# tigrazone/zig_raytracing_contest

Measured on AMD Instinct MI355X. Metric: Mrays/sec + wall-clock to output.png on contest config.json scene, higher is better.
Workload: dtype f32; 1 GPU; cfg3: contest stand-in (99480 tris, 553091 refs), 1920x1080, 256 spp, max_bounce 4, grid 128^3; global_batch=530841600, parallelism=tiles1, schedule=timed: default pass sets

## Files before the change

### zig_raytracing_contest_amd/csrc/render.hip

```cpp
#include <hip/hip_runtime.h>

#include <algorithm>
#include <cstdio>
#include <cstdlib>
#include <cstring>
#include <ctime>
#include <new>
#include <vector>

#include "zrt_internal.h"
#include "dda.h"
#include "escape.h"
#include "device_geometry.h"

using namespace zrt;

#define HIP_TRY(expr)                                                            \
    do {                                                                         \
        hipError_t _e = (expr);                                                  \
        if (_e != hipSuccess) {                                                  \
            if (getenv("ZRT_DEBUG"))                                             \
                fprintf(stderr, "zrt: %s failed: %s (%s:%d)\n", #expr,           \
                        hipGetErrorString(_e), __FILE__, __LINE__);              \
            return _e == hipErrorOutOfMemory ? ZRT_ERR_OUT_OF_MEMORY : ZRT_ERR_HIP; \
        }                                                                        \
    } while (0)

namespace {

constexpr float kFltEps = 1.1920928955078125e-07f;
constexpr int kBlock = 256;
constexpr int kTraceBlock = 512;
constexpr int kTraceThreads = 256;
#ifndef ZRT_TRI_BATCH
#define ZRT_TRI_BATCH 1
#endif
constexpr int kTriBatch = ZRT_TRI_BATCH;
#ifndef ZRT_PARK_BLOCK_T
#define ZRT_PARK_BLOCK_T 1024
#endif
constexpr int kParkBlock = ZRT_PARK_BLOCK_T;
#ifndef ZRT_SHADE_N
#define ZRT_SHADE_N 3
#endif
constexpr int kShadeEntries = ZRT_SHADE_N;
#ifndef ZRT_WF_CHUNK
#define ZRT_WF_CHUNK 3
#endif
constexpr uint32_t kWfChunk = ZRT_WF_CHUNK;

#ifndef ZRT_PLANES16
#define ZRT_PLANES16 1
#endif
#ifndef ZRT_ESCAPE
#define ZRT_ESCAPE 1
#endif
#ifndef ZRT_FRUSTUM
#define ZRT_FRUSTUM 1
#endif
#ifndef ZRT_FRUSTUM_HI
#define ZRT_FRUSTUM_HI 1
#endif
#ifndef ZRT_NORMALIZE_RN
#define ZRT_NORMALIZE_RN 1
#endif
#if ZRT_NORMALIZE_RN
#define ZRT_NORM_RN normalize_rn
#else
#define ZRT_NORM_RN normalize
#endif
#ifndef ZRT_FFN
#define ZRT_FFN 1
#endif
#ifndef ZRT_PRIMARY_BMASK
#define ZRT_PRIMARY_BMASK 1
#endif
#ifndef ZRT_WALK_FACE_SKIP
#define ZRT_WALK_FACE_SKIP 1
#endif
#ifndef ZRT_FAST_QUOT_WF
#define ZRT_FAST_QUOT_WF 1
#endif
#ifndef ZRT_FRUSTUM_SHIFT
#define ZRT_FRUSTUM_SHIFT 2
#endif
constexpr uint32_t kFrustShift = ZRT_FRUSTUM_SHIFT;
static_assert(kFrustShift <= 3, "a frustum block lies inside one tile (tile edges are multiples of 8)");
#ifndef ZRT_PACK_BM
#define ZRT_PACK_BM 1
#endif

constexpr double kFrustB = (double)(1u << ZRT_FRUSTUM_SHIFT);
#ifndef ZRT_WALK_STEPS
#define ZRT_WALK_STEPS 4
#endif
#ifndef ZRT_WALK_STEPS_NOESC
#define ZRT_WALK_STEPS_NOESC 5
#endif
constexpr uint32_t kTriFloats = 12u;

struct TraceParams {
    float bmin[3], bmax[3];
    uint32_t res[3];
    float cs[3];
    float ics[3];
    uint32_t cs_ok;
    const uint2* cells;
    const float* tri_pos;
    const float4* tri_data;
    const DevMat* mats;
    uint32_t nmat;
    const float* texels;
    const double* zig;
    const uint32_t* occ;
    uint32_t occ_shift, occ_nb0, occ_nb01, occ_words;
    const unsigned long long* bmask;
    const float4* tlo;
    uint32_t tlo_nbx;
    PackK pk;
    const uint32_t* cell32;
    uint32_t occ_o1, occ_o2, occ_w0, occ_w1, occ_w2, occ_lowm;
    uint32_t ox1, ox2, ow0, ow1, ow2;
    float org[3], llc[3], right[3], up[3];
    uint32_t w;
    const uint32_t* pixlist;
    uint32_t P;
    uint32_t s0;
    uint32_t total;
    uint32_t S;
    DivS sdiv;
    uint32_t max_bounce;
    uint64_t seed;
    float4* out;
    uint32_t* counter;
    unsigned long long* stats;
};

__device__ __forceinline__ void load_tri(const TraceParams& p, uint32_t j, v3& v0, v3& e1, v3& e2) {
    const float* q = p.tri_pos + (uint64_t)kTriFloats * j;
    const float4 a = *reinterpret_cast<const float4*>(q), b = *reinterpret_cast<const float4*>(q + 4),
                 c = *reinterpret_cast<const float4*>(q + 8);
    v0 = mk(a.x, a.y, a.z); e1 = mk(b.x, b.y, b.z); e2 = mk(c.x, c.y, c.z);
}

template <int N>
struct Stack {
    float e[3 * N], a[3 * N];
    uint32_t used;
    __device__ __forceinline__ void init() { used = 0u; }
    __device__ __forceinline__ void set(uint32_t slot, v3 ee, v3 aa) {
        e[3 * slot] = ee.x; e[3 * slot + 1] = ee.y; e[3 * slot + 2] = ee.z;
        a[3 * slot] = aa.x; a[3 * slot + 1] = aa.y; a[3 * slot + 2] = aa.z;
        used |= 1u << slot;
    }
    __device__ __forceinline__ v3 fold(v3 L) const {
        for (int i = N - 1; i >= 0; --i) {
            if ((used >> i) & 1u) {
                L = add(mk(e[3 * i], e[3 * i + 1], e[3 * i + 2]),
                        mul(mk(a[3 * i], a[3 * i + 1], a[3 * i + 2]), L));
            }
        }
        return L;
    }
};

__device__ __forceinline__ bool brick_occupied(const TraceParams& p, const uint32_t* occ, uint32_t c0,
                                               uint32_t c1, uint32_t c2) {
    const uint32_t s = p.occ_shift;
    const uint32_t b = __umul24(c2 >> s, p.occ_nb01) + __umul24(c1 >> s, p.occ_nb0) + (c0 >> s);
    return (occ[b >> 5] >> (b & 31u)) & 1u;
}

template <bool BM>
__device__ __forceinline__ bool brick_occupied_v(const TraceParams& p, const uint32_t* occ, uint32_t pc) {
    if (BM) {
        return __builtin_amdgcn_ubfe(occ[pc >> 11], pc >> 6, 1u);
    }
    const uint32_t b = __umul24(__builtin_amdgcn_ubfe(pc, p.occ_o2, p.occ_w2), p.occ_nb01) +
                       __umul24(__builtin_amdgcn_ubfe(pc, p.occ_o1, p.occ_w1), p.occ_nb0) +
                       __builtin_amdgcn_ubfe(pc, p.occ_shift, p.occ_w0);
    return (occ[b >> 5] >> (b & 31u)) & 1u;
}

template <bool BM>
__device__ __forceinline__ bool occx_cell(unsigned long long bm, const DdaV& s, const PackK& k) {
    if (BM) return (uint32_t)(bm >> (s.pc & 63u)) & 1u;
    const uint32_t i = __umul24(s.pc & k.low2, k.kmul) >> k.kshr;
    return (uint32_t)(bm >> (i & 63u)) & 1u;
}

__device__ __forceinline__ GridK grid_consts(const TraceParams& p) {
    GridK g;
    g.rm0 = __builtin_amdgcn_readfirstlane(p.res[0] - 1u);
    g.rm1 = __builtin_amdgcn_readfirstlane(p.res[1] - 1u);
    g.rm2 = __builtin_amdgcn_readfirstlane(p.res[2] - 1u);
    g.str1 = __builtin_amdgcn_readfirstlane(p.res[0]);
    g.str2 = __builtin_amdgcn_readfirstlane(p.res[0] * p.res[1]);
    return g;
}

__device__ __forceinline__ bool first_active_lane() {
    return (threadIdx.x & 63u) == (uint32_t)__builtin_ctzll(__ballot(1));
}

template <int TB, bool STATS, bool MTX = false>
__device__ __forceinline__ void test_cell(const TraceParams& p, uint32_t b, uint32_t e, v3 o, v3 d,
                                          float& nearest, float& hu, float& hv, uint32_t& hidx,
                                          uint32_t& n_tests, uint64_t* wstat) {
    for (uint32_t i = b; i < e; i += TB) {
        if (STATS && first_active_lane()) ++wstat[1];
        v3 A[TB], B[TB], Cc[TB];
#pragma unroll
        for (int k = 0; k < TB; ++k) load_tri(p, min(i + (uint32_t)k, e - 1u), A[k], B[k], Cc[k]);
#pragma unroll
        for (int k = 0; k < TB; ++k) {
            if (i + (uint32_t)k < e) {
                if (STATS) ++n_tests;
                float t, u, v;
                if (tri_ray<MTX>(A[k], B[k], Cc[k], o, d, &t, &u, &v)) {
                    if (nearest > t && t > 0.0f) { nearest = t; hu = u; hv = v; hidx = i + k; }
                }
            }
        }
    }
}

template <int TB, bool MTX>
__device__ __forceinline__ void test_cell_keep(const TraceParams& p, uint32_t b, uint32_t e, uint32_t keep, v3 o,
                                               v3 d, float& nearest, float& hu, float& hv, uint32_t& hidx) {
    const uint32_t cnt = e - b;
    if (cnt > 32u || keep == ~0u) {
        uint32_t dummy = 0;
        test_cell<TB, false, MTX>(p, b, e, o, d, nearest, hu, hv, hidx, dummy, nullptr);
        return;
    }
    uint32_t m = keep & ((cnt < 32u ? (1u << cnt) : 0u) - 1u);
    while (m) {
        uint32_t k[TB];
        bool has[TB];
#pragma unroll
        for (int j = 0; j < TB; ++j) {
            has[j] = m != 0u;
            k[j] = has[j] ? (uint32_t)__builtin_ctz(m) : k[0];
            m &= m - 1u;
        }
        v3 A[TB], B[TB], Cc[TB];
#pragma unroll
        for (int j = 0; j < TB; ++j) load_tri(p, b + k[j], A[j], B[j], Cc[j]);
#pragma unroll
        for (int j = 0; j < TB; ++j) {
            if (has[j]) {
                float t, u, v;
                if (tri_ray<MTX>(A[j], B[j], Cc[j], o, d, &t, &u, &v)) {
                    if (nearest > t && t > 0.0f) { nearest = t; hu = u; hv = v; hidx = b + k[j]; }
                }
            }
        }
    }
}

template <bool STATS, int TB, bool PACKED = false, bool PK_BM = false, bool MTX = false>
__device__ __forceinline__ float trace_ray(const TraceParams& p, const uint32_t* occ, v3 o, v3 d,
                                           float& hu, float& hv, uint32_t& hidx, uint32_t& n_cells,
                                           uint32_t& n_tests, uint64_t* prof, uint32_t* wcnt = nullptr,
                                           float tau = 0.0f, float tfar = kInf) {
    float nearest = kInf;
    Dda s0;
    if (ZRT_FAST_QUOT && ZRT_FAST_QUOT_WF && !MTX && !STATS) {
        if (!dda_init_fq(p.bmin, p.bmax, p.res, p.cs, p.ics, p.cs_ok != 0u, o, d, s0)) return nearest;
    } else if (!dda_init(p.bmin, p.bmax, p.res, p.cs, o, d, s0)) {
        return nearest;
    }
    const uint32_t sh = p.occ_shift;
    const GridK gk = grid_consts(p);
    if constexpr (PACKED) {
        static_assert(!STATS, "the counting build walks unpacked");
        DdaV s;
        ddav_from_t<PK_BM>(s0, gk, p.pk, s);
        uint32_t f0 = p.pk.f0, f1 = p.pk.f1, f2 = p.pk.f2;
        asm("" : "+s"(f0), "+s"(f1), "+s"(f2));
        if (ZRT_FRUSTUM && s0.neg < 8u) {
            if (tau == kInf) return nearest;
            if (tau > fminf(s.tn0, fminf(s.tn1, s.tn2))) {
                bool exited;
                if (ZRT_FFN) DDAV_FFN(s, p.pk, f0, f1, f2, tau, exited);
                else DDAV_FF4(s, f0, f1, f2, tau, exited);
                if (exited) return nearest;
            }
        }
        bool occupied = brick_occupied_v<PK_BM>(p, occ, s.pc);
        constexpr bool kBm = PK_BM && ZRT_PRIMARY_BMASK;
        unsigned long long q = 0ull;
        if (kBm && occupied) q = p.bmask[s.pc >> 6];
        float lim = ZRT_FRUSTUM_HI && s0.neg < 8u ? tfar : kInf;
        float tcl = __builtin_nanf("");
        for (;;) {
            if (kBm ? ((q >> (s.pc & 63u)) & 1ull) != 0ull : occupied) {
                const uint32_t* rec = p.cell32 + 8ull * s.pc;
                const uint2 cell = *reinterpret_cast<const uint2*>(rec);
                if (ZRT_WALK_FACE_SKIP) {
                    const bool x0 = s.tn0 == tcl + s.td0, x1 = s.tn1 == tcl + s.td1, x2 = s.tn2 == tcl + s.td2;
                    uint32_t keep = ~0u;
                    if ((uint32_t)x0 + (uint32_t)x1 + (uint32_t)x2 == 1u) {
                        const uint32_t face = x0 ? (s.d0 >> 31) : (x1 ? 2u + (s.d1 >> 31) : 4u + (s.d2 >> 31));
                        keep = rec[2 + face];
                    }
                    test_cell_keep<TB, MTX>(p, cell.x, cell.y, keep, o, d, nearest, hu, hv, hidx);
                } else {
                    test_cell<TB, false, MTX>(p, cell.x, cell.y, o, d, nearest, hu, hv, hidx, n_tests, prof);
                }
                lim = fminf(lim, nearest);
            }
            bool crossed, exited;
            float tc;
            PackK pkl = p.pk;
            pkl.f0 = f0; pkl.f1 = f1; pkl.f2 = f2;
            DDAV_STEPX(s, pkl, p.occ_lowm, crossed, exited, tc);
            if (exited || lim <= tc) break;
            tcl = tc;
            if (crossed) {
                occupied = brick_occupied_v<PK_BM>(p, occ, s.pc);
                if (kBm) q = occupied ? p.bmask[s.pc >> 6] : 0ull;
            }
        }
        return nearest;
    }
    DdaW s;
    ddaw_from(s0, gk, s);
    bool occupied = brick_occupied(p, occ, s.c0, s.c1, s.c2);
    for (;;) {
        if (STATS) ++n_cells;
        if (STATS && first_active_lane()) ++prof[8];
        uint32_t ncell = 0;
        if (occupied) {
            const uint2 cell = p.cells[s.lin];
            if (STATS) { prof[6] += 1; prof[7] += cell.y > cell.x ? 1 : 0; ncell = cell.y - cell.x; }
            test_cell<TB, STATS, MTX>(p, cell.x, cell.y, o, d, nearest, hu, hv, hidx, n_tests, prof + 8);
        }
        if (STATS) {
            uint32_t* wc = wcnt + 2 * (threadIdx.x >> 6);
            const bool first = first_active_lane();
            if (first) wc[0] = 0;
            __builtin_amdgcn_wave_barrier();
            atomicAdd(&wc[0], ncell);
            __builtin_amdgcn_wave_barrier();
            if (first) {
                const uint32_t N = wc[0];
                prof[10] += N ? 1 : 0;
                prof[4] += (N + 63) / 64;
            }
        }
        bool crossed;
        float t_exit;
        DDAW_STEP(s, sh, crossed, t_exit);
        if (nearest <= t_exit) break;
        if (crossed) occupied = brick_occupied(p, occ, s.c0, s.c1, s.c2);
    }
    return nearest;
}

#ifndef ZRT_TEX1
#define ZRT_TEX1 1
#endif
__device__ __forceinline__ v3 sample3(const float* texels, const DevTex& t, float u, float v) {
    const float* b = texels + t.off;
    if (ZRT_TEX1 && t.w == 1 && t.h == 1) {
        const float fu = tex_frac(u), fv = tex_frac(v);
        const float x = __int_as_float(t.umin), y = __int_as_float(t.umax), z = __int_as_float(t.vmin);
        return mk(bilerp(x, x, x, x, fu, fv), bilerp(y, y, y, y, fu, fv), bilerp(z, z, z, z, fu, fv));
    }
    const TexCoords c = tex_coords(t.w, t.h, t.umin, t.umax, t.vmin, t.vmax, u, v);
    v3 r;
    r.x = bilerp(b[3 * c.i11 + 0], b[3 * c.i21 + 0], b[3 * c.i12 + 0], b[3 * c.i22 + 0], c.fu, c.fv);
    r.y = bilerp(b[3 * c.i11 + 1], b[3 * c.i21 + 1], b[3 * c.i12 + 1], b[3 * c.i22 + 1], c.fu, c.fv);
    r.z = bilerp(b[3 * c.i11 + 2], b[3 * c.i21 + 2], b[3 * c.i12 + 2], b[3 * c.i22 + 2], c.fu, c.fv);
    return r;
}
__device__ __forceinline__ float sample1(const float* texels, const DevTex& t, float u, float v) {
    const float* b = texels + t.off;
    if (ZRT_TEX1 && t.w == 1 && t.h == 1) {
        const float x = __int_as_float(t.umin);
        return bilerp(x, x, x, x, tex_frac(u), tex_frac(v));
    }
    const TexCoords c = tex_coords(t.w, t.h, t.umin, t.umax, t.vmin, t.vmax, u, v);
    return bilerp(b[c.i11], b[c.i21], b[c.i12], b[c.i22], c.fu, c.fv);
}

__device__ __forceinline__ unsigned long long wave_sum(unsigned long long x) {
#pragma unroll
    for (int off = 32; off > 0; off >>= 1) {
        const unsigned lo = __shfl_xor((unsigned)x, off);
        const unsigned hi = __shfl_xor((unsigned)(x >> 32), off);
        x += ((unsigned long long)hi << 32) | lo;
    }
    return x;
}

__device__ __forceinline__ void camera_ray(const TraceParams& p, uint32_t item, Rng& rng, v3& o, v3& d,
                                           uint32_t* block = nullptr) {
    const uint32_t q = div_by(item, p.sdiv);
    const uint32_t s_local = item - q * p.S;
    const uint32_t pixel = p.pixlist[q];
    const uint32_t py = pixel / p.w;
    const uint32_t px = pixel - py * p.w;
    if (block) *block = (py >> kFrustShift) * p.tlo_nbx + (px >> kFrustShift);
    rng.s = path_key(p.seed, pixel, p.s0 + s_local);
    const float jx = rng_float(rng);
    const float jy = rng_float(rng);
    o = mk(p.org[0], p.org[1], p.org[2]);
    d = ZRT_NORM_RN(add(add(mk(p.llc[0], p.llc[1], p.llc[2]),
                          scale(mk(p.right[0], p.right[1], p.right[2]), (float)px + jx)),
                      scale(mk(p.up[0], p.up[1], p.up[2]), (float)py + jy)));
}

__device__ __forceinline__ Rng camera_rng(const TraceParams& p, uint32_t item) {
    const uint32_t q = div_by(item, p.sdiv);
    const uint32_t s_local = item - q * p.S;
    const uint32_t pixel = p.pixlist[q];
    Rng rng;
    rng.s = path_key(p.seed, pixel, p.s0 + s_local);
    (void)rng_float(rng);
    (void)rng_float(rng);
    return rng;
}

template <int MAXB>
__global__ __launch_bounds__(kTraceBlock, 1) void trace_kernel(const TraceParams p) {
    __shared__ double s_zig[514];
    extern __shared__ __attribute__((aligned(16))) uint32_t s_occ[];
    uint64_t prof[11] = {0, 0, 0, 0, 0, 0, 0, 0, 0, 0, 0};
    __shared__ uint32_t s_wcnt[2 * (kTraceBlock / 64)];
    for (uint32_t i = threadIdx.x; i < 514; i += blockDim.x) s_zig[i] = p.zig[i];
    for (uint32_t i = threadIdx.x; i < p.occ_words; i += blockDim.x) s_occ[i] = p.occ[i];
    __syncthreads();
    const double* zx = s_zig;
    const double* zf = s_zig + 257;

    const uint32_t lane = threadIdx.x & 63u;
    uint32_t n_seg = 0, n_cells = 0, n_tests = 0, n_hits = 0;
    uint32_t p_seg = 0, p_cells = 0, p_tests = 0, p_hits = 0;

    for (;;) {
        uint32_t base = 0;
        if (lane == 0) base = atomicAdd(p.counter, 64u);
        base = __builtin_amdgcn_readfirstlane(base);
        if (base >= p.total) break;
        const uint32_t item = base + lane;
        if (item >= p.total) continue;

        Rng rng;
        v3 o, d;
        camera_ray(p, item, rng, o, d);
        Stack<MAXB> stk;
        stk.init();
        v3 L = mk(0, 0, 0);
        uint32_t slot = 0;
        for (uint32_t depth = p.max_bounce; depth > 0; --depth, ++slot) {
            ++n_seg;
            float hu = 0.0f, hv = 0.0f;
            uint32_t hidx = 0;
            const uint32_t c_before = n_cells, t_before = n_tests;
            const float t = trace_ray<true, kTriBatch, false, false, true>(p, s_occ, o, d, hu, hv, hidx, n_cells,
                                                                           n_tests, prof, s_wcnt);
            if (slot == 0) { ++p_seg; p_cells += n_cells - c_before; p_tests += n_tests - t_before; }
            if (t == kInf) { L = env_color(d); break; }
            ++n_hits;
            if (slot == 0) ++p_hits;
            const float4* tdp = p.tri_data + 4ull * hidx;
            const float4 d0 = tdp[0], d1 = tdp[1], d2 = tdp[2], d3 = tdp[3];
            const float w0 = 1.0f - hu - hv;
            const float tc0 = (d2.y * w0 + d2.w * hu) + d3.y * hv;
            const float tc1 = (d2.z * w0 + d3.x * hu) + d3.z * hv;
            const DevMat& m = p.mats[__float_as_uint(d3.w)];
            const v3 albedo = sample3(p.texels, m.tex[0], tc0, tc1);
            const v3 emissive = sample3(p.texels, m.tex[1], tc0, tc1);
            const float transparency = sample1(p.texels, m.tex[2], tc0, tc1);
            const v3 nrm = add(add(scale(mk(d0.x, d0.y, d0.z), w0), scale(mk(d0.w, d1.x, d1.y), hu)),
                               scale(mk(d1.z, d1.w, d2.x), hv));
            const v3 no = add(o, scale(d, t + kFltEps));
            if (!(rng_float(rng) > transparency)) {
                const float nx = (float)rng_norm64(rng, zx, zf);
                const float ny = (float)rng_norm64(rng, zx, zf);
                const float nz = (float)rng_norm64(rng, zx, zf);
                d = normalize(add(nrm, normalize(mk(nx, ny, nz))));
                stk.set(slot, emissive, albedo);
            }
            o = no;
        }
        L = stk.fold(L);
        p.out[item] = make_float4(L.x, L.y, L.z, 0.0f);
    }
    const unsigned long long s0 = wave_sum(n_seg), s1 = wave_sum(n_cells), s2 = wave_sum(n_tests),
                             s3 = wave_sum(n_hits), s4 = wave_sum(prof[6]), s5 = wave_sum(prof[7]),
                             s6 = wave_sum(prof[8]), s7 = wave_sum(prof[9]), s8 = wave_sum(prof[10]),
                             s9 = wave_sum(prof[4]);
    const unsigned long long q0 = wave_sum(p_seg), q1 = wave_sum(p_cells), q2 = wave_sum(p_tests),
                             q3 = wave_sum(p_hits);
    if (lane == 0) {
        atomicAdd(&p.stats[8], q0);
        atomicAdd(&p.stats[9], q1);
        atomicAdd(&p.stats[10], q2);
        atomicAdd(&p.stats[11], q3);
        atomicAdd(&p.stats[0], s0);
        atomicAdd(&p.stats[1], s1);
        atomicAdd(&p.stats[2], s2);
        atomicAdd(&p.stats[3], s3);
        atomicAdd(&p.stats[4], s4);
        atomicAdd(&p.stats[5], s5);
        atomicAdd(&p.stats[6], s6);
        atomicAdd(&p.stats[7], s7);
        atomicAdd(&p.stats[14], s8);
        atomicAdd(&p.stats[15], s9);
    }
}

struct WfParams {
    TraceParams t;
    const float4* q_in;
    float4* q_out;
    float4* stk4;
    float2* stk2;
    float4* term;
    uint32_t T;
    uint32_t* fetch8;
    const uint32_t* n_in8;
    uint32_t* n_out8;
    float4* hit;
    uint32_t* fetch8s;
    const uint32_t* occx;
    uint32_t occx_words, occx_nbw, occx_moff, occx_nb0, occx_nb01;
    uint32_t occx_ldsw;
    uint32_t test_min;
    uint32_t refill_min;
    uint32_t rel_min;
    uint32_t rel_emin;
    const uint32_t* esc;
    const uint32_t* bfc;
    uint64_t bfc_ones;
};

constexpr uint32_t kCtr = 32;

__device__ __forceinline__ uint32_t xcd_q0(uint32_t P, uint32_t g) {
    const uint32_t nblk = (P + 63u) >> 6;
    return min(P, (nblk * g / 8u) * 64u);
}

__device__ __forceinline__ uint32_t region_base(const WfParams& w, uint32_t g) { return w.t.S * xcd_q0(w.t.P, g); }

#ifdef ZRT_SWEEP
#define SHADE_STAMP(k, v) do { if (sp) { asm volatile("" :: "v"(v)); const uint64_t t_ = __builtin_amdgcn_s_memtime(); \
    const uint32_t n_ = (uint32_t)__popcll(__ballot(1)); \
    if (first_active_lane()) { sp[k] += t_ - sp[16]; sp[16] = t_; sp[8 + (k)] += n_; } } } while (0)
#else
#define SHADE_STAMP(k, v) do { (void)sp; } while (0)
#endif
struct TriRec {
    float4 d0, d1, d2, d3;
};
__device__ __forceinline__ TriRec tri_rec(const TraceParams& p, float t, uint32_t hidx) {
    TriRec r;
    if (t == kInf) {
        r.d0 = r.d1 = r.d2 = r.d3 = make_float4(0.0f, 0.0f, 0.0f, 0.0f);
        return r;
    }
    const float4* tdp = p.tri_data + 4ull * hidx;
    r.d0 = tdp[0]; r.d1 = tdp[1]; r.d2 = tdp[2]; r.d3 = tdp[3];
    return r;
}
template <bool LAST = false>
__device__ __forceinline__ bool shade_segment(const WfParams& w, const double* zx, const double* zf,
                                              const DevMat* mats, uint32_t item, float t, float hu, float hv,
                                              const TriRec& tr, v3& o, v3& d, uint32_t& depth, uint32_t& slot,
                                              Rng& rng, uint32_t& mask, v3& L,
                                              unsigned long long* sp = nullptr) {
    SHADE_STAMP(1, t);
    if (t == kInf) { L = env_color(d); return false; }
    const TraceParams& p = w.t;
    const float4 d0 = tr.d0, d1 = tr.d1, d2 = tr.d2, d3 = tr.d3;
    const float w0 = 1.0f - hu - hv;
    const float tc0 = (d2.y * w0 + d2.w * hu) + d3.y * hv;
    const float tc1 = (d2.z * w0 + d3.x * hu) + d3.z * hv;
    SHADE_STAMP(2, tc1);
    const DevMat& m = mats[__float_as_uint(d3.w)];
    const v3 albedo = sample3(p.texels, m.tex[0], tc0, tc1);
    const v3 emissive = sample3(p.texels, m.tex[1], tc0, tc1);
    const float transparency = sample1(p.texels, m.tex[2], tc0, tc1);
    SHADE_STAMP(3, transparency);
    const v3 nrm = add(add(scale(mk(d0.x, d0.y, d0.z), w0), scale(mk(d0.w, d1.x, d1.y), hu)),
                       scale(mk(d1.z, d1.w, d2.x), hv));
    const v3 no = add(o, scale(d, t + kFltEps));
    const float u_tr = rng_float(rng);
    SHADE_STAMP(4, u_tr);
    if (LAST) {
        L = !(u_tr > transparency) ? add(emissive, mul(albedo, mk(0.0f, 0.0f, 0.0f))) : mk(0, 0, 0);
        return false;
    }
    if (!(u_tr > transparency)) {
        if (ZRT_PLANES16) {
            const uint32_t eb = __float_as_uint(emissive.x) | __float_as_uint(emissive.y) | __float_as_uint(emissive.z);
            w.stk4[(uint64_t)slot * w.T + item] = make_float4(albedo.x, albedo.y, albedo.z, __uint_as_float(eb));
            if (eb != 0u)
                reinterpret_cast<float4*>(w.stk2)[(uint64_t)slot * w.T + item] =
                    make_float4(emissive.x, emissive.y, emissive.z, 0.0f);
        } else {
            w.stk4[(uint64_t)slot * w.T + item] = make_float4(emissive.x, emissive.y, emissive.z, albedo.x);
            w.stk2[(uint64_t)slot * w.T + item] = make_float2(albedo.y, albedo.z);
        }
        const float nx = (float)rng_norm64(rng, zx, zf);
        const float ny = (float)rng_norm64(rng, zx, zf);
        const float nz = (float)rng_norm64(rng, zx, zf);
        d = ZRT_NORM_RN(add(nrm, ZRT_NORM_RN(mk(nx, ny, nz))));
        mask |= 1u << slot;
        SHADE_STAMP(5, d.x);
    }
    o = no;
    --depth;
    ++slot;
    L = mk(0, 0, 0);
    return depth != 0;
}

__device__ __forceinline__ void q_store(const WfParams& w, uint32_t pos, v3 o, v3 d, uint32_t item, uint32_t depth,
                                        uint32_t slot, const Rng& rng, uint32_t mask) {
    w.q_out[3ull * pos] = make_float4(o.x, o.y, o.z, __uint_as_float(item));
    w.q_out[3ull * pos + 1] = make_float4(d.x, d.y, d.z, __uint_as_float(depth | (slot << 16)));
    w.q_out[3ull * pos + 2] = make_float4(__uint_as_float((uint32_t)rng.s), __uint_as_float((uint32_t)(rng.s >> 32)),
                                          __uint_as_float(mask), 0.0f);
}

__device__ __forceinline__ void wf_append(const WfParams& w, bool cont, uint64_t below, v3 o, v3 d, uint32_t item,
                                          uint32_t depth, uint32_t slot, const Rng& rng, uint32_t mask,
                                          uint32_t reg) {
    uint64_t pend = __ballot(cont);
    while (pend) {
        const uint32_t lead = (uint32_t)__builtin_ctzll(pend);
        const uint32_t g = (uint32_t)__builtin_amdgcn_readlane((int)reg, (int)lead);
        const uint64_t m = __ballot(cont && reg == g);
        uint32_t ob = 0;
        if ((threadIdx.x & 63u) == lead) ob = atomicAdd(&w.n_out8[g * kCtr], (uint32_t)__popcll(m));
        ob = (uint32_t)__builtin_amdgcn_readlane((int)ob, (int)lead) + region_base(w, g);
        if (cont && reg == g) q_store(w, ob + (uint32_t)__popcll(m & below), o, d, item, depth, slot, rng, mask);
        pend &= ~m;
    }
}

template <bool PRIMARY>
__device__ __forceinline__ bool wf_fetch(const WfParams& w, uint32_t want, uint32_t& grp, uint32_t& tried,
                                         uint32_t& base, uint32_t& lim) {
    const TraceParams& p = w.t;
    const uint32_t S = p.S;
    for (;;) {
        const uint32_t q0 = xcd_q0(p.P, grp);
        const uint32_t pg = xcd_q0(p.P, grp + 1u) - q0;
        lim = PRIMARY ? S * pg : w.n_in8[grp * kCtr];
        uint32_t b = 0;
        if ((threadIdx.x & 63u) == 0) b = atomicAdd(&w.fetch8[grp * kCtr], want);
        base = __builtin_amdgcn_readfirstlane(b);
        if (base < lim) return true;
        if (++tried == 8u) return false;
        grp = (grp + 1u) & 7u;
    }
}
template <bool PRIMARY>
__device__ __forceinline__ uint32_t ent_index(const WfParams& w, uint32_t grp, uint32_t j) {
    return region_base(w, grp) + j;
}

template <bool PRIMARY>
__device__ __forceinline__ void path_state(const WfParams& w, uint32_t i, uint32_t& item, uint32_t& depth,
                                           uint32_t& slot, Rng& rng, uint32_t& mask) {
    if (PRIMARY) {
        item = i;
        depth = w.t.max_bounce;
        slot = 0;
        mask = 0;
        rng = camera_rng(w.t, i);
    } else {
        const float4 a = w.q_in[3ull * i], b = w.q_in[3ull * i + 1], c = w.q_in[3ull * i + 2];
        item = __float_as_uint(a.w);
        depth = __float_as_uint(b.w) & 0xFFFFu;
        slot = __float_as_uint(b.w) >> 16;
        rng.s = ((uint64_t)__float_as_uint(c.y) << 32) | __float_as_uint(c.x);
        mask = __float_as_uint(c.z);
    }
}

template <int MINW, bool PRIMARY, bool PACKED, bool PK_BM = false, bool MTX = false>
__global__ __launch_bounds__(kTraceBlock, MINW) void wf_kernel(const WfParams w) {
    const TraceParams& p = w.t;
    __shared__ double s_zig[514];
    extern __shared__ __attribute__((aligned(16))) uint32_t s_occ[];
    for (uint32_t i = threadIdx.x; i < 514; i += blockDim.x) s_zig[i] = p.zig[i];
    for (uint32_t i = threadIdx.x; i < p.occ_words; i += blockDim.x) s_occ[i] = p.occ[i];
    __syncthreads();
    const double* zx = s_zig;
    const double* zf = s_zig + 257;
    const uint32_t lane = threadIdx.x & 63u;
    const uint64_t below = lane ? (~0ull >> (64u - lane)) : 0ull;
    uint32_t n_seg = 0, dummy = 0;
    uint32_t grp = blockIdx.x & 7u, tried = 0;
#ifdef ZRT_SWEEP
    unsigned long long wprof[3] = {0, 0, 0};
    uint64_t wtick = __builtin_amdgcn_s_memtime();
#define WF_STAMP(k) do { const uint64_t t_ = __builtin_amdgcn_s_memtime(); wprof[k] += t_ - wtick; wtick = t_; } while (0)
#else
#define WF_STAMP(k) do { } while (0)
#endif

    for (;;) {
        uint32_t base = 0, lim = 0;
        if (!wf_fetch<PRIMARY>(w, 64u * kWfChunk, grp, tried, base, lim)) break;
      for (uint32_t sub = 0; sub < kWfChunk && base + 64u * sub < lim; ++sub) {
        const uint32_t j = base + 64u * sub + lane;
        const bool valid = j < lim;
        const uint32_t i = valid ? ent_index<PRIMARY>(w, grp, j) : 0u;
        bool cont = false;
        uint32_t mask = 0, r_item = 0, r_depth = 0, r_slot = 0;
        v3 r_o = mk(0, 0, 0), r_d = mk(0, 0, 0);
        Rng r_rng;
        r_rng.s = 0;
        if (valid) {
            v3 o, d;
            uint32_t depth;
            float tau = 0.0f, tfar = kInf;
            if (PRIMARY) {
                Rng rng0;
                uint32_t blk = 0;
                camera_ray(p, i, rng0, o, d, &blk);
                if (ZRT_FRUSTUM && p.tlo) {
                    const float4 fb = p.tlo[blk];
                    tau = fb.x;
                    tfar = fb.y;
                }
                depth = p.max_bounce;
            } else {
                const float4 a = w.q_in[3ull * i], b = w.q_in[3ull * i + 1];
                o = mk(a.x, a.y, a.z);
                d = mk(b.x, b.y, b.z);
                depth = __float_as_uint(b.w) & 0xFFFFu;
            }
            float t = kInf, hu = 0.0f, hv = 0.0f;
            uint32_t hidx = 0;
            WF_STAMP(2);
            if (depth != 0)
                t = trace_ray<false, kTriBatch, PACKED, PK_BM, MTX>(p, s_occ, o, d, hu, hv, hidx, dummy, dummy, nullptr,
                                                                    nullptr, tau, tfar);
            WF_STAMP(0);
            uint32_t item, slot;
            Rng rng;
            path_state<PRIMARY>(w, i, item, depth, slot, rng, mask);
            v3 L = mk(0, 0, 0);
            if (depth != 0) {
                ++n_seg;
                cont = shade_segment(w, zx, zf, p.mats, item, t, hu, hv, tri_rec(p, t, hidx), o, d, depth, slot, rng,
                                     mask, L);
            }
            if (!cont) w.term[item] = make_float4(L.x, L.y, L.z, __uint_as_float(mask));
            r_item = item; r_depth = depth; r_slot = slot; r_o = o; r_d = d; r_rng = rng;
            WF_STAMP(1);
        }
        wf_append(w, cont, below, r_o, r_d, r_item, r_depth, r_slot, r_rng, mask, grp);
        WF_STAMP(2);
      }
    }
    const unsigned long long s0 = wave_sum(n_seg);
    if (lane == 0) atomicAdd(&p.stats[0], s0);
#ifdef ZRT_SWEEP
    if (PRIMARY && lane == 0)
        for (int k = 0; k < 3; ++k) atomicAdd(&p.stats[29 + k], wprof[k]);
#endif
#undef WF_STAMP
}

struct OccX {
    const uint2* ent;
    const unsigned long long* masks;
};
__device__ __forceinline__ unsigned long long occx_mask_at(const OccX& L, uint2 e, uint32_t b) {
    const uint32_t low = __builtin_amdgcn_ubfe(e.x, 0u, b);
    const uint32_t bit = __builtin_amdgcn_ubfe(e.x, b, 1u);
    return L.masks[__umul24((uint32_t)__popc(low) + e.y, bit)];
}

__device__ __forceinline__ unsigned long long occx_mask(const OccX& L, uint32_t b) {
    return occx_mask_at(L, L.ent[b >> 5], b);
}
__device__ __forceinline__ unsigned long long occx_mask_clamped(const OccX& L, uint32_t b, uint32_t nbw) {
    return occx_mask_at(L, L.ent[min(b >> 5, nbw - 1u)], b);
}
__device__ __forceinline__ unsigned long long occx_mask_bm(const OccX& L, uint32_t pc) {
    return occx_mask_at(L, L.ent[pc >> 11], pc >> 6);
}
template <bool BM>
__device__ __forceinline__ uint32_t occx_brick(const WfParams& w, const DdaV& s) {
    if (BM) return s.pc >> 6;
    const TraceParams& p = w.t;
    return __umul24(__builtin_amdgcn_ubfe(s.pc, p.ox2, p.ow2), w.occx_nb01) +
           __umul24(__builtin_amdgcn_ubfe(s.pc, p.ox1, p.ow1), w.occx_nb0) + __builtin_amdgcn_ubfe(s.pc, 2u, p.ow0);
}

constexpr int kParkWaves = kParkBlock / 64;
#ifndef ZRT_PARK_CHUNK
#define ZRT_PARK_CHUNK 256
#endif
constexpr uint32_t kParkChunk = ZRT_PARK_CHUNK;
#ifndef ZRT_PARK_LATE_DRAIN
#define ZRT_PARK_LATE_DRAIN 1
#endif
#ifndef ZRT_PARK_QPF
#define ZRT_PARK_QPF 0
#endif
#ifndef ZRT_PARK_ADAPT
#define ZRT_PARK_ADAPT 1
#endif
__device__ __forceinline__ void park_load_range(const TraceParams& p, uint32_t pc, uint32_t* rng) {
    const uint32_t* c = p.cell32 + 8ull * pc;
    const uint32_t m0 = __builtin_amdgcn_readfirstlane((uint32_t)(uintptr_t)rng);
    asm volatile("s_mov_b32 m0, %2\n\t"
                 "global_load_lds_dword %0, off\n\t"
                 "s_add_u32 m0, m0, 0x100\n\t"
                 "global_load_lds_dword %1, off"
                 :
                 : "v"(c), "v"(c + 1), "s"(m0)
                 : "memory");
}
__device__ __forceinline__ void park_load_masked(const TraceParams& p, uint32_t pc, const uint32_t* mask,
                                                 uint32_t* rng) {
    const uint32_t* c = p.cell32 + 8ull * pc;
    const uint32_t m0 = __builtin_amdgcn_readfirstlane((uint32_t)(uintptr_t)rng);
    asm volatile("s_mov_b32 m0, %3\n\t"
                 "global_load_lds_dword %0, off\n\t"
                 "s_add_u32 m0, m0, 0x100\n\t"
                 "global_load_lds_dword %1, off\n\t"
                 "s_add_u32 m0, m0, 0x100\n\t"
                 "global_load_lds_dword %2, off"
                 :
                 : "v"(c), "v"(c + 1), "v"(mask), "s"(m0)
                 : "memory");
}
__device__ __forceinline__ void park_load_cell(const TraceParams& p, uint32_t pc, uint32_t face, uint32_t* rng) {
    park_load_masked(p, pc, p.cell32 + 8ull * pc + 2 + face, rng);
}

__device__ __forceinline__ void park_load_esc(const uint32_t* word, uint32_t* esc) {
    const uint32_t m0 = __builtin_amdgcn_readfirstlane((uint32_t)(uintptr_t)esc);
    asm volatile("s_mov_b32 m0, %1\n\t"
                 "global_load_lds_dword %0, off"
                 :
                 : "v"(word), "s"(m0)
                 : "memory");
}

struct ParkSlot {
    float4 o[64];
    float4 d[64];
    unsigned long long best[64];
    float2 uv[64];
    uint32_t mark[64];
};

__device__ __forceinline__ uint32_t wave_excl_sum(uint32_t x, uint32_t lane, uint32_t& total) {
    uint32_t s = x;
    s += (uint32_t)__builtin_amdgcn_update_dpp(0, (int)s, 0x111, 0xf, 0xf, true);
    s += (uint32_t)__builtin_amdgcn_update_dpp(0, (int)s, 0x112, 0xf, 0xf, true);
    s += (uint32_t)__builtin_amdgcn_update_dpp(0, (int)s, 0x114, 0xf, 0xf, true);
    s += (uint32_t)__builtin_amdgcn_update_dpp(0, (int)s, 0x118, 0xf, 0xf, true);
    const uint32_t r0 = (uint32_t)__builtin_amdgcn_readlane((int)s, 15);
    const uint32_t r1 = (uint32_t)__builtin_amdgcn_readlane((int)s, 31);
    const uint32_t r2 = (uint32_t)__builtin_amdgcn_readlane((int)s, 47);
    const uint32_t r3 = (uint32_t)__builtin_amdgcn_readlane((int)s, 63);
    const uint32_t row = lane >> 4;
    s += row == 0u ? 0u : (row == 1u ? r0 : (row == 2u ? r0 + r1 : r0 + r1 + r2));
    total = r0 + r1 + r2 + r3;
    return s - x;
}

#ifdef ZRT_SWEEP
#define PARK_PROF_DECL unsigned long long pprof[21] = {0, 0, 0, 0, 0, 0, 0, 0, 0, 0, 0, 0, 0, 0, 0, 0, 0, 0, 0, 0, 0}; \
    uint64_t ptick = __builtin_amdgcn_s_memtime();
#define PARK_STAMP(k) do { const uint64_t t_ = __builtin_amdgcn_s_memtime(); pprof[k] += t_ - ptick; ptick = t_; } while (0)
#define PARK_COUNT(k, v) (pprof[k] += (v))
#else
#define PARK_PROF_DECL
#define PARK_STAMP(k) do { } while (0)
#define PARK_COUNT(k, v) do { } while (0)
#endif

#ifndef ZRT_PARK_WPE
#define ZRT_PARK_WPE 5
#endif
#if ZRT_PARK_WPE
#define ZRT_PARK_ATTR __attribute__((amdgpu_waves_per_eu(ZRT_PARK_WPE, 8)))
#else
#define ZRT_PARK_ATTR
#endif
template <bool ESC, bool PK_BM>
__global__ __launch_bounds__(kParkBlock) ZRT_PARK_ATTR void wf_park_kernel(const WfParams w) {
    const TraceParams& p = w.t;
    extern __shared__ __attribute__((aligned(16))) uint32_t s_dyn[];
    __shared__ uint32_t s_rng[kParkWaves * 192];
    uint32_t* const rng_slot = s_rng + 192u * (threadIdx.x >> 6);
    __shared__ uint32_t s_esc[kParkWaves * 64];
    uint32_t* const esc_slot = s_esc + 64u * (threadIdx.x >> 6);
// ... 1953 lines not shown
        zrt_context::PassSet& ps = c->set[k];
        if ((rc = grow(&ps.q0, &ps.q0_cap, 3 * T)) != ZRT_OK) return rc;
        if ((rc = grow(&ps.q1, &ps.q1_cap, 3 * T)) != ZRT_OK) return rc;
        if ((rc = grow(&ps.term, &ps.term_cap, T)) != ZRT_OK) return rc;
        if ((rc = grow(&ps.stk4, &ps.stk4_cap, T * nb)) != ZRT_OK) return rc;
        if ((rc = grow(&ps.stk2, &ps.stk2_cap, T * nb * (ZRT_PLANES16 ? 2 : 1))) != ZRT_OK) return rc;
        if ((rc = grow(&ps.wfc, &ps.wfc_cap, 32ull * kCtr * (mb + 2))) != ZRT_OK) return rc;
        if (k == 0) {
            ps.stream = c->stream;
        } else {
            if (!ps.stream) HIP_TRY(hipStreamCreateWithFlags(&ps.stream, hipStreamNonBlocking));
            if (!ps.ev_join) HIP_TRY(hipEventCreateWithFlags(&ps.ev_join, hipEventDisableTiming));
        }
    }
    if (nsets > 1) {
        if (!c->ev_fork) HIP_TRY(hipEventCreateWithFlags(&c->ev_fork, hipEventDisableTiming));
        while (c->ev_pass.size() < npasses) {
            hipEvent_t e;
            HIP_TRY(hipEventCreateWithFlags(&e, hipEventDisableTiming));
            c->ev_pass.push_back(e);
        }
    }
    if (npasses > 1 && (rc = grow(&c->d_acc, &c->acc_cap, P)) != ZRT_OK) return rc;
    if ((rc = grow(&c->d_rgb, &c->rgb_cap, 3ull * P)) != ZRT_OK) return rc;
    const bool want_lin = outs && outs->linear_packed;
    if (want_lin && (rc = grow(&c->d_lin, &c->lin_cap, 3ull * P)) != ZRT_OK) return rc;
    const uint32_t launches_per_pass = counting ? 1 : nb;
    while (c->ev_trace.size() < 2ull * npasses * launches_per_pass) {
        hipEvent_t e;
        HIP_TRY(hipEventCreate(&e));
        c->ev_trace.push_back(e);
    }

    const size_t nk = ktimes ? (size_t)npasses * (2 * nb + 1) : 0;
    while (c->ev_k.size() < 2 * nk) {
        hipEvent_t e;
        HIP_TRY(hipEventCreate(&e));
        c->ev_k.push_back(e);
    }
    c->ev_k_cls.assign(nk, 0);

    const bool mtx = c->mt_exact || (cfg->flags & ZRT_FLAG_MT_EXACT);
    const bool park_next = c->occx_ok && !counting && !(cfg->flags & ZRT_FLAG_LANE_WALK) &&
                           c->packed && !mtx;
    const bool rel = !(cfg->flags & ZRT_FLAG_NO_RELEASE) && (c->rel_on || (cfg->flags & ZRT_FLAG_RELEASE));
    uint32_t test_min = rel ? kParkTestMinRel : kParkTestMin, refill_min = kParkRefillMin;
#if defined(ZRT_SWEEP) || defined(ZRT_SETS_ENV)
    if (const char* e = getenv("ZRT_PARK_T")) test_min = (uint32_t)std::max(1, std::min(64, atoi(e)));
    if (const char* e = getenv("ZRT_PARK_R")) refill_min = (uint32_t)std::max(1, std::min(64, atoi(e)));
#endif
    uint32_t rel_min = test_min;
    uint32_t rel_emin = 1;
#if defined(ZRT_SWEEP) || defined(ZRT_SETS_ENV)
    if (const char* e = getenv("ZRT_PARK_REL")) rel_min = (uint32_t)std::max(1, std::min(64, atoi(e)));
    if (const char* e = getenv("ZRT_PARK_REL_E")) rel_emin = (uint32_t)std::max(1, std::min(64, atoi(e)));
#endif
    const bool packed = c->packed && !mtx;
    const bool pbm = packed && c->pk.bm;
    const WfFn f_first = mtx ? kWfPrimaryExact : packed ? (pbm ? kWfPrimaryBM : kWfPrimary) : kWfPrimaryWide;
    if (!c->esc_tried && park_next && !(cfg->flags & ZRT_FLAG_NO_ESCAPE) && (big || (cfg->flags & ZRT_FLAG_ESCAPE))) {
        c->esc_tried = true;
        if ((rc = context_escape(c)) != ZRT_OK) return rc;
    }
    const bool esc = c->d_esc && !(cfg->flags & ZRT_FLAG_NO_ESCAPE) &&
                     (c->esc_on || (cfg->flags & ZRT_FLAG_ESCAPE));
    if (park_next && !(cfg->flags & ZRT_FLAG_NO_BFCULL)) {
        const bool forced = (cfg->flags & ZRT_FLAG_BFCULL) != 0;
        if (forced ? !c->bfc_tried_forced : (big && !c->bfc_tried)) {
            c->bfc_tried = true;
            c->bfc_tried_forced = c->bfc_tried_forced || forced;
            if ((rc = context_bfcull(c, forced)) != ZRT_OK) return rc;
        }
    }
    const bool bfc = c->d_bfc && !(cfg->flags & ZRT_FLAG_NO_BFCULL) && (c->bfc_on || (cfg->flags & ZRT_FLAG_BFCULL));
    const WfFn f_next = park_next ? (pbm ? (esc ? (WfFn)wf_park_kernel<true, true> : (WfFn)wf_park_kernel<false, true>)
                                         : (esc ? (WfFn)wf_park_kernel<true, false> : (WfFn)wf_park_kernel<false, false>))
                                  : mtx ? kWfBounceExact : (packed ? (pbm ? kWfBounceBM : kWfBounce) : kWfBounceWide);
    const WfFn s_next = c->nmat <= kLdsMats ? (WfFn)wf_shade_kernel<true> : (WfFn)wf_shade_kernel<false>;
    const WfFn s_last = !ZRT_SHADE_LAST ? s_next
                        : c->nmat <= kLdsMats ? (WfFn)wf_shade_kernel<true, true> : (WfFn)wf_shade_kernel<false, true>;
    const size_t lds_shade = c->nmat <= kLdsMats ? c->nmat * sizeof(DevMat) : 0;
    for (uint32_t k = 0; k < nsets && park_next; ++k)
        if ((rc = grow(&c->set[k].hit, &c->set[k].hit_cap, T)) != ZRT_OK) return rc;

    {
        auto shortfall = [&](const char* what, const void* ptr, size_t cap, uint64_t need) {
            if (ptr && cap >= need) return false;
            if (getenv("ZRT_DEBUG"))
                fprintf(stderr, "zrt: capacity guard: %s holds %zu, the launch writes %llu\n", what, ptr ? cap : 0,
                        (unsigned long long)need);
            return true;
        };
        bool bad = shortfall("pixel list", c->d_pix, c->pix_cap, P) || shortfall("rgb", c->d_rgb, c->rgb_cap, 3ull * P) ||
                   (npasses > 1 && shortfall("accumulator", c->d_acc, c->acc_cap, P)) ||
                   (want_lin && shortfall("linear", c->d_lin, c->lin_cap, 3ull * P)) ||
                   (counting && shortfall("counting output", c->d_out, c->out_cap, T));
        for (uint32_t k = 0; k < nsets && !counting && !bad; ++k) {
            const zrt_context::PassSet& ps = c->set[k];
            bad = shortfall("q0", ps.q0, ps.q0_cap, 3 * T) || shortfall("q1", ps.q1, ps.q1_cap, 3 * T) ||
                  shortfall("term", ps.term, ps.term_cap, T) || shortfall("planes4", ps.stk4, ps.stk4_cap, T * nb) ||
                  shortfall("planes2", ps.stk2, ps.stk2_cap, T * nb * (ZRT_PLANES16 ? 2 : 1)) ||
                  shortfall("counters", ps.wfc, ps.wfc_cap, 32ull * kCtr * (mb + 2)) ||
                  (park_next && shortfall("hit records", ps.hit, ps.hit_cap, T)) ||
                  (k > 0 && (!ps.stream || !ps.ev_join));
        }
        for (uint32_t pass = 0; pass < npasses && !bad; ++pass)
            bad = (uint64_t)pass_count(pass) * P > T || pass_first(pass) + pass_count(pass) > spp;
        if (bad) return ZRT_ERR_INVALID_ARG;
    }

    const size_t lds_wf = 4ull * c->occ_words;
    int park_block = kParkBlock;
#ifdef ZRT_SWEEP
    if (const char* e = getenv("ZRT_PARK_BLOCK")) park_block = std::max(64, std::min(kParkBlock, atoi(e) / 64 * 64));
#endif
    const uint32_t occx_ldsw = (uint32_t)occx_lds_words(c->occx_nbw, c->occx_moff, c->occx_words);
    const size_t lds_park = 4ull * occx_ldsw + (size_t)(park_block / 64) * sizeof(ParkSlot);
    if (getenv("ZRT_WF_DEBUG"))
        fprintf(stderr, "{\"zrt_park_lds\": {\"occx_bytes\": %u, \"block\": %d, \"lds_per_block\": %zu, "
                "\"release_frac\": %.4f, \"release\": %d}}\n",
                4u * occx_ldsw, park_block, lds_park, c->rel_frac, rel ? 1 : 0);
    auto grid_for = [&](const void* f, int threads, size_t lds, uint32_t* blocks) -> int {
        int bpc = 0;
        HIP_TRY(hipFuncSetAttribute(f, hipFuncAttributeMaxDynamicSharedMemorySize, (int)lds));
        HIP_TRY(hipOccupancyMaxActiveBlocksPerMultiprocessor(&bpc, f, threads, lds));
        if (getenv("ZRT_WF_DEBUG"))
            fprintf(stderr, "{\"zrt_grid\": {\"threads\": %d, \"lds\": %zu, \"blocks_per_cu\": %d}}\n", threads, lds, bpc);
        bpc = std::max(1, std::min(bpc, 2048 / threads));
        *blocks = (uint32_t)(c->num_cus * bpc);
        return ZRT_OK;
    };
    uint32_t grid_first = 0, grid_next = 0, grid_count = 0, grid_shade = 0, grid_shade_last = 0;
    const int thr_first = kTraceThreads;
    const int thr_next = park_next ? park_block : kTraceThreads;
    const size_t lds_first = lds_wf, lds_next = park_next ? lds_park : lds_wf;
    if (counting) {
        if ((rc = grid_for((const void*)cfn, kTraceThreads, lds_wf, &grid_count)) != ZRT_OK) return rc;
    } else {
        if ((rc = grid_for((const void*)f_first, thr_first, lds_first, &grid_first)) != ZRT_OK) return rc;
        if ((rc = grid_for((const void*)f_next, thr_next, lds_next, &grid_next)) != ZRT_OK) return rc;
        if ((rc = grid_for((const void*)s_next, kTraceThreads, lds_shade, &grid_shade)) != ZRT_OK) return rc;
        if ((rc = grid_for((const void*)s_last, kTraceThreads, lds_shade, &grid_shade_last)) != ZRT_OK) return rc;
    }

    TraceParams tp;
    scene_params(c, tp);
    for (int i = 0; i < 3; ++i) {
        tp.org[i] = cam->origin[i];
        tp.llc[i] = cam->lower_left_corner[i];
        tp.right[i] = cam->right[i];
        tp.up[i] = cam->up[i];
    }
    tp.w = cam->w;
    tp.pixlist = c->d_pix;
    tp.P = P;
    tp.max_bounce = mb;
    tp.seed = cfg->seed;
    tp.out = c->d_out;
    tp.counter = c->d_counter;
    tp.stats = c->d_stats;
    const float inv_spp = 1.0f / (float)spp;
    size_t kn = 0;
    auto kt_begin = [&](int cls, hipStream_t sm) -> int {
        if (!ktimes) return ZRT_OK;
        c->ev_k_cls[kn] = (uint8_t)cls;
        HIP_TRY(hipEventRecord(c->ev_k[2 * kn], sm));
        return ZRT_OK;
    };
    auto kt_end = [&](hipStream_t sm) -> int {
        if (!ktimes) return ZRT_OK;
        HIP_TRY(hipEventRecord(c->ev_k[2 * kn + 1], sm));
        ++kn;
        return ZRT_OK;
    };
    zrt_kernel_profile kp{};

    HIP_TRY(hipMemsetAsync(c->d_stats, 0, 512, c->stream));
    HIP_TRY(hipEventRecord(c->ev_begin, c->stream));
    if (ZRT_FRUSTUM && c->d_sat && !counting && packed && !(cfg->flags & ZRT_FLAG_NO_FRUSTUM) &&
        ((uint64_t)P * cfg->num_samples >= kFrustumMinSamples || (cfg->flags & ZRT_FLAG_FRUSTUM))) {
        const uint32_t nbx = (cam->w + (1u << kFrustShift) - 1u) >> kFrustShift;
        const uint32_t nby = (cam->h + (1u << kFrustShift) - 1u) >> kFrustShift;
        if ((rc = grow(&c->d_tlo, &c->tlo_cap, (size_t)nbx * nby)) != ZRT_OK) return rc;
        FrustumArgs fa;
        for (int k = 0; k < 3; ++k) {
            fa.res[k] = c->grid.resolution[k];
            fa.bmin[k] = c->grid.bbox_min[k];
            fa.bmax[k] = c->grid.bbox_max[k];
            fa.cs[k] = c->grid.cell_size[k];
            fa.org[k] = cam->origin[k];
            fa.llc[k] = cam->lower_left_corner[k];
            fa.right[k] = cam->right[k];
            fa.up[k] = cam->up[k];
        }
        fa.w = cam->w; fa.h = cam->h; fa.nbx = nbx; fa.nby = nby;
        const uint32_t tile = cfg->tile_size ? cfg->tile_size : 64u;
        fa.tb = tile >> kFrustShift;
        fa.tx = (cam->w + tile - 1u) / tile;
        fa.rank = cfg->rank;
        fa.nranks = nranks;
        const uint64_t ntiles = (uint64_t)fa.tx * ((cam->h + tile - 1u) / tile);
        const uint64_t per_tile = (ntiles - cfg->rank + nranks - 1u) / nranks * fa.tb * fa.tb;
        fa.whole = per_tile > (uint64_t)nbx * nby ? 1u : 0u;
        const uint64_t fthreads = (fa.whole ? (uint64_t)nbx * nby : per_tile) * 64u;
        hipLaunchKernelGGL(frustum_kernel, dim3((uint32_t)((fthreads + kBlock - 1) / kBlock)), dim3(kBlock), 0, c->stream,
                           (const uint32_t*)c->d_sat, fa, c->d_tlo);
        HIP_TRY(hipGetLastError());
        tp.tlo = c->d_tlo;
        tp.tlo_nbx = nbx;
    }
    if (nsets > 1) {
        HIP_TRY(hipEventRecord(c->ev_fork, c->stream));
        for (uint32_t k = 1; k < nsets; ++k) HIP_TRY(hipStreamWaitEvent(c->set[k].stream, c->ev_fork, 0));
    }
    uint32_t launches = 0, ne = 0;
    for (uint32_t pass = 0; pass < npasses; ++pass) {
        const zrt_context::PassSet& ps = c->set[counting ? 0u : pass % nsets];
        hipStream_t sm = counting ? c->stream : ps.stream;
        float4* const q0 = ps.q0;
        float4* const q1 = ps.q1;
        float4* const term = ps.term;
        float4* const stk4 = ps.stk4;
        float2* const stk2 = ps.stk2;
        uint32_t* const wfc = ps.wfc;
        float4* const hit = ps.hit;
        const uint32_t s0 = pass_first(pass);
        const uint32_t S = pass_count(pass);
        tp.s0 = s0;
        tp.total = S * P;
        tp.S = S;
        tp.sdiv = div_magic(S);
        const int first = pass == 0 ? 1 : 0, last = pass + 1 == npasses ? 1 : 0;
        if (!counting) {
            HIP_TRY(hipMemsetAsync(wfc, 0, 4ull * 32 * kCtr * (mb + 2), sm));
            WfParams W;
            memset(&W, 0, sizeof W);
            W.t = tp;
            W.stk4 = stk4;
            W.stk2 = stk2;
            W.term = term;
            W.T = (uint32_t)T;
            W.occx = c->d_occx;
            W.occx_words = c->occx_words;
            W.occx_ldsw = occx_ldsw;
            W.occx_nbw = c->occx_nbw;
            W.occx_moff = c->occx_moff;
            W.occx_nb0 = c->occx_nb[0];
            W.occx_nb01 = c->occx_nb[0] * c->occx_nb[1];
            W.test_min = test_min;
            W.refill_min = refill_min;
            W.rel_min = rel ? rel_min : 0u;
            W.rel_emin = rel_emin;
            W.esc = c->d_esc;
            W.bfc = bfc ? c->d_bfc : nullptr;
            W.bfc_ones = c->bfc_bytes ? c->bfc_bytes / 4 - 1 : 0;
            for (uint32_t k = 0; k < nb; ++k) {
                W.q_in = (k & 1) ? q0 : q1;
                W.q_out = (k & 1) ? q1 : q0;
                W.fetch8 = wfc + kCtr * (16 * k);
                W.n_in8 = wfc + kCtr * (16 * k + 8);
                W.n_out8 = wfc + kCtr * (16 * (k + 1) + 8);
                W.hit = hit;
                W.fetch8s = wfc + kCtr * (16 * (mb + 2) + 8 * k);
                HIP_TRY(hipEventRecord(c->ev_trace[ne++], sm));
                const int cls = k == 0 ? ZRT_KERNEL_PRIMARY : (park_next ? ZRT_KERNEL_PARK : ZRT_KERNEL_BOUNCE);
                if ((rc = kt_begin(cls, sm)) != ZRT_OK) return rc;
                if (k == 0)
                    hipLaunchKernelGGL(f_first, dim3(grid_first), dim3(thr_first), lds_first, sm, W);
                else
                    hipLaunchKernelGGL(f_next, dim3(grid_next), dim3(thr_next), lds_next, sm, W);
                HIP_TRY(hipGetLastError());
                if ((rc = kt_end(sm)) != ZRT_OK) return rc;
                ++kp.launches[cls];
                if (k > 0 && park_next) {
                    if ((rc = kt_begin(ZRT_KERNEL_SHADE, sm)) != ZRT_OK) return rc;
                    if (k + 1 == nb)
                        hipLaunchKernelGGL(s_last, dim3(grid_shade_last), dim3(kTraceThreads), lds_shade, sm, W);
                    else
                        hipLaunchKernelGGL(s_next, dim3(grid_shade), dim3(kTraceThreads), lds_shade, sm, W);
                    HIP_TRY(hipGetLastError());
                    if ((rc = kt_end(sm)) != ZRT_OK) return rc;
                    ++kp.launches[ZRT_KERNEL_SHADE];
                }
                HIP_TRY(hipEventRecord(c->ev_trace[ne++], sm));
                ++launches;
            }
            if (nsets > 1 && pass > 0) HIP_TRY(hipStreamWaitEvent(sm, c->ev_pass[pass - 1], 0));
            if ((rc = kt_begin(ZRT_KERNEL_RESOLVE, sm)) != ZRT_OK) return rc;
            hipLaunchKernelGGL(wf_resolve_kernel, dim3((P + kResPix - 1) / kResPix), dim3(kBlock), 0, sm,
                               term, stk4, stk2, (uint32_t)T, P, S, mb, c->d_acc, first, last, inv_spp,
                               c->d_rgb, want_lin ? c->d_lin : nullptr);
            if ((rc = kt_end(sm)) != ZRT_OK) return rc;
            ++kp.launches[ZRT_KERNEL_RESOLVE];
            if (nsets > 1) HIP_TRY(hipEventRecord(c->ev_pass[pass], sm));
        } else {
            HIP_TRY(hipMemsetAsync(c->d_counter, 0, 4, c->stream));
            HIP_TRY(hipEventRecord(c->ev_trace[ne++], c->stream));
            if ((rc = kt_begin(ZRT_KERNEL_COUNT, c->stream)) != ZRT_OK) return rc;
            hipLaunchKernelGGL(cfn, dim3(grid_count), dim3(kTraceThreads), lds_wf, c->stream, tp);
            HIP_TRY(hipGetLastError());
            if ((rc = kt_end(c->stream)) != ZRT_OK) return rc;
            ++kp.launches[ZRT_KERNEL_COUNT];
            ++launches;
            HIP_TRY(hipEventRecord(c->ev_trace[ne++], c->stream));
            if ((rc = kt_begin(ZRT_KERNEL_RESOLVE, c->stream)) != ZRT_OK) return rc;
            hipLaunchKernelGGL(resolve_kernel, dim3((P + kBlock - 1) / kBlock), dim3(kBlock), 0, c->stream,
// ... 877 lines not shown
```

Baseline: 7221 Mrays/s.

## Compute primary camera rays per wave with uniform loads and reuse RNG state

When samples per pixel are at least 64, the primary wavefront kernel resolves each wave's contiguous item range to at most two pixels. It fetches their pixel indices and frustum bounds with scalar uniform loads instead of per-lane gathers. It also swaps the pixel-row division for a magic-number divide. The RNG state after camera jitter is kept in a register (or shared memory in mode 1) rather than recomputed by camera_rng after tracing. Together these trim per-lane integer divides, hashing and divergent memory loads on the primary path, at the cost of more live registers across trace_ray.

```diff
diff --git a/zig_raytracing_contest_amd/csrc/render.hip b/zig_raytracing_contest_amd/csrc/render.hip
--- a/zig_raytracing_contest_amd/csrc/render.hip
+++ b/zig_raytracing_contest_amd/csrc/render.hip
@@ -83,6 +83,9 @@
 #endif
 #ifndef ZRT_FRUSTUM_SHIFT
 #define ZRT_FRUSTUM_SHIFT 2
+#endif
+#ifndef ZRT_PRIMARY_RNG
+#define ZRT_PRIMARY_RNG 2
 #endif
 constexpr uint32_t kFrustShift = ZRT_FRUSTUM_SHIFT;
 static_assert(kFrustShift <= 3, "a frustum block lies inside one tile (tile edges are multiples of 8)");
@@ -123,6 +126,7 @@
     uint32_t ox1, ox2, ow0, ow1, ow2;
     float org[3], llc[3], right[3], up[3];
     uint32_t w;
+    DivS wdiv;
     const uint32_t* pixlist;
     uint32_t P;
     uint32_t s0;
@@ -396,21 +400,70 @@
     return x;
 }
 
-__device__ __forceinline__ void camera_ray(const TraceParams& p, uint32_t item, Rng& rng, v3& o, v3& d,
-                                           uint32_t* block = nullptr) {
+struct CamPix {
+    uint32_t pixel, s_local;
+    float fx, fy;
+};
+__device__ __forceinline__ void pixel_xy(const TraceParams& p, uint32_t pixel, uint32_t& px, uint32_t& py) {
+    py = p.wdiv.m ? div_by(pixel, p.wdiv) : pixel / p.w;
+    px = pixel - py * p.w;
+}
+__device__ __forceinline__ uint32_t frustum_block(const TraceParams& p, uint32_t px, uint32_t py) {
+    return (py >> kFrustShift) * p.tlo_nbx + (px >> kFrustShift);
+}
+__device__ __forceinline__ CamPix camera_pixel(const TraceParams& p, uint32_t item, uint32_t* block = nullptr) {
     const uint32_t q = div_by(item, p.sdiv);
-    const uint32_t s_local = item - q * p.S;
-    const uint32_t pixel = p.pixlist[q];
-    const uint32_t py = pixel / p.w;
-    const uint32_t px = pixel - py * p.w;
-    if (block) *block = (py >> kFrustShift) * p.tlo_nbx + (px >> kFrustShift);
-    rng.s = path_key(p.seed, pixel, p.s0 + s_local);
+    CamPix c;
+    c.s_local = item - q * p.S;
+    c.pixel = p.pixlist[q];
+    uint32_t px, py;
+    pixel_xy(p, c.pixel, px, py);
+    if (block) *block = frustum_block(p, px, py);
+    c.fx = (float)px;
+    c.fy = (float)py;
+    return c;
+}
+__device__ __forceinline__ void camera_ray(const TraceParams& p, const CamPix& c, Rng& rng, v3& o, v3& d) {
+    rng.s = path_key(p.seed, c.pixel, p.s0 + c.s_local);
     const float jx = rng_float(rng);
     const float jy = rng_float(rng);
     o = mk(p.org[0], p.org[1], p.org[2]);
     d = ZRT_NORM_RN(add(add(mk(p.llc[0], p.llc[1], p.llc[2]),
-                          scale(mk(p.right[0], p.right[1], p.right[2]), (float)px + jx)),
-                      scale(mk(p.up[0], p.up[1], p.up[2]), (float)py + jy)));
+                          scale(mk(p.right[0], p.right[1], p.right[2]), c.fx + jx)),
+                      scale(mk(p.up[0], p.up[1], p.up[2]), c.fy + jy)));
+}
+__device__ __forceinline__ void camera_ray(const TraceParams& p, uint32_t item, Rng& rng, v3& o, v3& d) {
+    camera_ray(p, camera_pixel(p, item), rng, o, d);
+}
+
+template <class T>
+__device__ __forceinline__ T uniform_load(const T* ptr) {
+    return *(const __attribute__((address_space(4))) T*)ptr;
+}
+
+__device__ __forceinline__ CamPix camera_pixel_wave(const TraceParams& p, uint32_t i0, uint32_t nv, uint32_t lane,
+                                                    float& tau, float& tfar) {
+    const uint32_t qa = div_by(i0, p.sdiv), qb = div_by(i0 + nv - 1u, p.sdiv);
+    const uint32_t sa = i0 - qa * p.S;
+    const uint32_t pa = uniform_load(p.pixlist + qa), pb = uniform_load(p.pixlist + qb);
+    uint32_t xa, ya, xb, yb;
+    pixel_xy(p, pa, xa, ya);
+    pixel_xy(p, pb, xb, yb);
+    const bool second = sa + lane >= p.S;
+    if (ZRT_FRUSTUM && p.tlo) {
+        const float* fa = reinterpret_cast<const float*>(p.tlo + frustum_block(p, xa, ya));
+        const float* fb = reinterpret_cast<const float*>(p.tlo + frustum_block(p, xb, yb));
+        const float lo_a = uniform_load(fa), hi_a = uniform_load(fa + 1);
+        const float lo_b = uniform_load(fb), hi_b = uniform_load(fb + 1);
+        tau = second ? lo_b : lo_a;
+        tfar = second ? hi_b : hi_a;
+    }
+    CamPix c;
+    c.s_local = sa + lane - (second ? p.S : 0u);
+    c.pixel = second ? pb : pa;
+    c.fx = second ? (float)xb : (float)xa;
+    c.fy = second ? (float)yb : (float)ya;
+    return c;
 }
 
 __device__ __forceinline__ Rng camera_rng(const TraceParams& p, uint32_t item) {
@@ -691,6 +744,7 @@
     const TraceParams& p = w.t;
     __shared__ double s_zig[514];
     extern __shared__ __attribute__((aligned(16))) uint32_t s_occ[];
+    __shared__ volatile unsigned long long s_rng[PRIMARY && ZRT_PRIMARY_RNG == 1 ? kTraceThreads : 1];
     for (uint32_t i = threadIdx.x; i < 514; i += blockDim.x) s_zig[i] = p.zig[i];
     for (uint32_t i = threadIdx.x; i < p.occ_words; i += blockDim.x) s_occ[i] = p.occ[i];
     __syncthreads();
@@ -724,16 +778,26 @@
             v3 o, d;
             uint32_t depth;
             float tau = 0.0f, tfar = kInf;
+            Rng rng0;
+            rng0.s = 0;
             if (PRIMARY) {
-                Rng rng0;
-                uint32_t blk = 0;
-                camera_ray(p, i, rng0, o, d, &blk);
-                if (ZRT_FRUSTUM && p.tlo) {
-                    const float4 fb = p.tlo[blk];
-                    tau = fb.x;
-                    tfar = fb.y;
+                CamPix cp;
+                if (p.S >= 64u) {
+                    const uint32_t j0 = __builtin_amdgcn_readfirstlane(base + 64u * sub);
+                    cp = camera_pixel_wave(p, __builtin_amdgcn_readfirstlane(ent_index<PRIMARY>(w, grp, j0)),
+                                           __builtin_amdgcn_readfirstlane(min(64u, lim - j0)), lane, tau, tfar);
+                } else {
+                    uint32_t blk = 0;
+                    cp = camera_pixel(p, i, &blk);
+                    if (ZRT_FRUSTUM && p.tlo) {
+                        const float4 fb = p.tlo[blk];
+                        tau = fb.x;
+                        tfar = fb.y;
+                    }
                 }
+                camera_ray(p, cp, rng0, o, d);
                 depth = p.max_bounce;
+                if (ZRT_PRIMARY_RNG == 1) s_rng[threadIdx.x] = rng0.s;
             } else {
                 const float4 a = w.q_in[3ull * i], b = w.q_in[3ull * i + 1];
                 o = mk(a.x, a.y, a.z);
@@ -749,7 +813,15 @@
             WF_STAMP(0);
             uint32_t item, slot;
             Rng rng;
-            path_state<PRIMARY>(w, i, item, depth, slot, rng, mask);
+            if (PRIMARY && ZRT_PRIMARY_RNG != 0) {
+                item = i;
+                depth = p.max_bounce;
+                slot = 0;
+                mask = 0;
+                rng.s = ZRT_PRIMARY_RNG == 1 ? s_rng[threadIdx.x] : rng0.s;
+            } else {
+                path_state<PRIMARY>(w, i, item, depth, slot, rng, mask);
+            }
             v3 L = mk(0, 0, 0);
             if (depth != 0) {
                 ++n_seg;
@@ -3009,6 +3081,7 @@
         tp.up[i] = cam->up[i];
     }
     tp.w = cam->w;
+    if ((uint64_t)cam->w * cam->h <= 0x80000000ull) tp.wdiv = div_magic(cam->w);
     tp.pixlist = c->d_pix;
     tp.P = P;
     tp.max_bounce = mb;
```

New measurement: 7249 Mrays/s (median of 6 runs). No clear change (+0.4%).
